# RobinVogel/Trade-offs-in-Distributed-Tuplewise-Estimation-and-Learning

Hardware: AMD Instinct MI355X
Metric: pair comparisons/sec (node) for sharded AUC U-stat at n=1e6/class (UnN, N=64 prop-SWOR shards, device repartition each step) (higher is better)
Workload: dtype f64

## Files before the change

include/tuplewise.h:

```cpp
#ifndef TUPLEWISE_H
#define TUPLEWISE_H

#include <stdint.h>

#ifdef __cplusplus
extern "C" {
#endif

#define TW_OK 0
#define TW_ERR_ARG 1
#define TW_ERR_HIP 2

#define TW_F64 0
#define TW_I64 1

#define TW_PRED_GT 0
#define TW_PRED_HALF 1
#define TW_PRED_SUBGT 2

#define TW_KERN_PROD 0
#define TW_KERN_GINI 1
#define TW_KERN_HINGE 2
#define TW_KERN_LOGISTIC 3

// ... 47 lines not shown
                  int32_t steps, int64_t x_shard, int64_t z_shard, int32_t n_shards,
                  void* d_x_bag, void* d_z_bag, uint32_t* d_cursors, uint64_t* d_send,
                  int64_t cap, int32_t* d_flag, void* stream);
int tw_chain_emit_ws(const uint64_t* d_x_rec, int64_t n_x, const uint64_t* d_z_rec, int64_t n_z,
                     int32_t half, uint32_t* d_x_pos, uint32_t* d_z_pos, int32_t first,
                     int32_t rank, int32_t world, const uint64_t* keys_x, const uint64_t* keys_z,
                     int32_t steps, int64_t x_shard, int64_t z_shard, int32_t n_shards,
                     void* d_x_bag, void* d_z_bag, uint32_t* d_cursors, uint64_t* d_send,
                     int64_t cap, int32_t* d_flag, void* d_work, int64_t work_bytes,
                     void* stream);
int64_t tw_chain_emit_work_bytes(int32_t steps, int64_t NX, int64_t NZ);
int32_t tw_chain_set_emit_tables(int32_t mode);
int32_t tw_chain_emit_tables_of(int64_t n_x, int64_t n_z, int32_t world, int32_t half,
                                int32_t exchange, int32_t n_shards);
int tw_chain_unpack(const uint64_t* d_recv, int32_t world, int32_t steps, int64_t cap,
                    int32_t half, int64_t n_x, int64_t n_z, int64_t x_shard, int64_t z_shard,
                    int32_t n_shards, void* d_x_bag, void* d_z_bag, uint32_t* d_cursors,
                    int32_t* d_flag, void* stream);
int tw_count_pairs_chain(const void* d_x_bag, const int64_t* d_x_off, int64_t x_stride,
                         const void* d_z_bag, const int64_t* d_z_off, int64_t z_stride,
                         int32_t n_shards, int32_t steps, int64_t max_nx, int64_t max_nz,
                         int32_t half, uint64_t* d_out, void* stream);
int tw_count_pairs_chain_planes(const void* d_x_bag, const int64_t* d_x_off, int64_t x_stride,
                                const void* d_z_bag, const int64_t* d_z_off, int64_t z_stride,
                                int32_t n_shards, int32_t steps, int64_t max_nx, int64_t max_nz,
                                int32_t half, int64_t image_bound, uint64_t* d_out,
                                void* stream, void* d_work, int64_t work_bytes);
int64_t tw_chain_planes_work_bytes(int32_t n_shards, int32_t steps, int64_t max_nx,
                                   int64_t max_nz, int32_t half, int64_t image_bound);
int32_t tw_count_chain_class_form(int32_t nb, int32_t k);
int32_t tw_count_chain_class_span(int32_t runs);
int32_t tw_count_chain_class_digits(int32_t w);
int32_t tw_count_chain_class_digits_of(int32_t nb, int32_t k);
int32_t tw_count_chain_prepass(int32_t mode);
int32_t tw_count_chain_prepass_of(int32_t n_shards, int32_t steps, int64_t max_nx,
                                  int64_t max_nz, int64_t image_bound);
int tw_count_pairs_chain_bucket(const void* d_x_bag, const int64_t* d_x_off, int64_t x_stride,
                                const void* d_z_bag, const int64_t* d_z_off, int64_t z_stride,
                                int32_t n_shards, int32_t steps, int64_t max_nz,
                                int64_t z_total, int32_t half, uint64_t* d_out, void* stream);
int tw_chain_set_emit(int32_t epr, int32_t steps_per_round);
int tw_count_chain_set_plan(int32_t R, int64_t z_chunk);
int tw_count_chain_set_swap(int32_t swap);
int tw_count_chain_set_class_bits(int32_t k);
int tw_chain_scatter(const void* d_x, const uint32_t* d_x_pos, int64_t n_x, const void* d_z,
                     const uint32_t* d_z_pos, int64_t n_z, void* d_x_out, void* d_z_out,
                     void* stream);

int64_t tw_count_pairs_sorted_work_bytes(int32_t n_shards, int64_t max_nz);
int tw_count_sorted_set_chunk(int64_t cap);
int tw_count_pairs_sorted(const void* d_x, const int64_t* d_x_off, const void* d_z,
                          const int64_t* d_z_off, int32_t n_shards, int64_t max_nx,
                          int64_t max_nz, int32_t dtype, int32_t pred, void* d_work,
                          uint64_t* d_out, void* stream);
int64_t tw_pair_moments_work_bytes(int32_t n_shards, int64_t total_nx, int64_t total_nz);
int tw_pair_moments(const void* d_x, const int64_t* d_x_off, const void* d_z,
                    const int64_t* d_z_off, int32_t n_shards, int64_t max_nx, int64_t max_nz,
                    int32_t dtype, int32_t pred, void* d_work, uint64_t* d_out, void* stream);
#define TW_MOMENTS_SORTED_MIN_PAIRS (1 << 17)
int tw_pair_moments_set_algo(int32_t algo);

int tw_count_pairs_sorted_step(const void* d_x, const int64_t* d_x_off, const void* d_z,
                               const int64_t* d_z_off, int32_t n_shards, int64_t max_nx,
                               int64_t max_nz, int32_t dtype, int32_t pred, void* d_work,
                               uint64_t* d_out, int64_t n_x, void* d_x_next, uint64_t key_x,
                               int64_t n_z, void* d_z_next, uint64_t key_z,
// ... 469 lines not shown
```

trade-offs-in-distributed-tuplewise-estimation-and-learning_amd/_lib.py:

```python
from __future__ import annotations

import ctypes
import os
import pathlib
import sys

import numpy as np

_HERE = pathlib.Path(__file__).resolve().parent
LIB_PATH = pathlib.Path(os.environ["TW_LIB_PATH"]) if os.environ.get("TW_LIB_PATH") else (
    _HERE / "libtuplewise.so")

TW_OK, TW_ERR_ARG, TW_ERR_HIP = 0, 1, 2
TW_F64, TW_I64 = 0, 1
TW_PRED_GT, TW_PRED_HALF, TW_PRED_SUBGT = 0, 1, 2
TW_KERN_PROD, TW_KERN_GINI, TW_KERN_HINGE, TW_KERN_LOGISTIC = 0, 1, 2, 3
TW_LOSS_HINGE, TW_LOSS_LOGISTIC = 0, 1
TW_SELF_GINI, TW_SELF_VAR, TW_SELF_KENDALL = 0, 1, 2
TW_MMD_GAUSSIAN, TW_MMD_ENERGY = 0, 1
TW_HSIC_GAUSSIAN, TW_HSIC_DISTANCE = 0, 1
TW_DIST_WITHIN, TW_DIST_CROSS = 0, 1

_vp, _i64, _i32, _u64, _f64 = (ctypes.c_void_p, ctypes.c_int64, ctypes.c_int32,
                               ctypes.c_uint64, ctypes.c_double)
# ... 194 lines not shown
    "tw_words_checksum": [_vp, _i64, _vp, _i64, _vp, _vp, _vp, _i64, _i64, _vp],
    "tw_words_checksum_acc_words": [],
    "tw_np_shuffle_pair": [_vp, _vp, _vp, _i64, _i64, _vp, _i64, _i64, _vp],
    "tw_np_shuffle_draws32": [_vp, _vp, _i64, _vp],
    "tw_np_shuffle_draws32_range": [_vp, _vp, _i64, _i64, _i64, _vp],
    "tw_shuffle_swaps_work_bytes": [_i64, _i64],
    "tw_shuffle_swaps_rounds": [_i64, _i64],
    "tw_shuffle_swaps_set_rounds": [_i32],
    "tw_shuffle_swaps_set_tail": [_i32],
    "tw_shuffle_swaps": [_vp, _i64, _vp, _i64, _vp, _vp, _i32, _i32, _vp, _vp, _vp],
    "tw_shuffle_swaps_windows": [],
    "tw_shuffle_swaps_part": [_vp, _i64, _vp, _i64, _vp, _vp, _i32, _i32, _i32, _vp, _vp, _vp],
    "tw_mt_minpoly": [_vp],
    "tw_mt_jump_poly": [_i64, _vp],
    "tw_mt_poly_mulmod": [_vp, _vp, _vp],
    "tw_mt_jump_host": [_vp, _vp, _i64],
    "tw_mt_states": [_vp, _i32, _vp, _i32, _vp, _vp],
    "tw_mt_generate": [_vp, _i32, _i32, _i32, _vp, _vp, _vp, _vp, _vp],
    "tw_np_randint_dev_work_bytes": [_i32, _i32, _i32, _i32],
    "tw_np_randint_dev": [_vp, _vp, _vp, _i32, _i32, _i32, _vp, _vp, _vp, _vp, _i32, _vp, _vp,
                          _vp, _i64, _vp, _vp, _vp],
    "tw_self_pairs_work_bytes": [_i32, _i64],
    "tw_self_pairs_idx_work_bytes": [_i32, _i64],
    "tw_self_pairs_tile": [],
    "tw_self_pairs": [_vp, _vp, _i32, _i64, _i32, _i32, _vp, _vp, _vp],
    "tw_self_pairs_idx32": [_vp, _vp, _vp, _vp, _i32, _i64, _i32, _i32, _vp, _vp, _vp],
    "tw_self_sorted_work_bytes": [_i32, _i64, _i64, _i32, _i32],
    "tw_self_sorted_chunk": [],
    "tw_self_sorted": [_vp, _vp, _i32, _i64, _i64, _i32, _i32, _i32, _vp, _vp, _vp],
    "tw_count_chain_class_form": [_i32, _i32],
    "tw_count_chain_class_span": [_i32],
    "tw_count_chain_class_digits": [_i32],
    "tw_count_chain_class_digits_of": [_i32, _i32],
    "tw_count_chain_prepass": [_i32],
    "tw_count_chain_prepass_of": [_i32, _i32, _i64, _i64, _i64],
    "tw_triplet_rows_tile": [],
    "tw_triplet_rows": [_vp, _vp, _i32, _vp, _vp, _i32, _i32, _i64, _i64, _i64, _i64, _vp, _vp,
                        _vp, _vp, _vp],
    "tw_triplet_idx_work_bytes": [_i32, _i64],
    "tw_triplet_idx32": [_vp, _vp, _i32, _vp, _vp, _vp, _vp, _i32, _i64, _i32, _vp, _vp, _vp],
    "tw_triplet_grad_tile": [],
    "tw_triplet_grad_work_bytes": [_i32, _i64, _i32, _i32],
    "tw_triplet_grad": [_vp, _vp, _i32, _vp, _i32, _vp, _vp, _vp, _vp, _i32, _i64, _f64, _i32, _vp,
                        _vp, _vp, _vp, _vp],
    "tw_triplet_project": [_vp, _i64, _i32, _vp, _i32, _vp, _vp],
    "tw_triplet_sgd_update": [_vp, _vp, _vp, _i32, _f64, _f64, _i32, _vp],
    "tw_mmd_tile": [],
    "tw_mmd_work_bytes": [_i32, _i64, _i64],
    "tw_mmd_idx_work_bytes": [_i32, _i64],
    "tw_mmd_sums": [_vp, _vp, _i32, _vp, _vp, _i32, _i64, _i64, _i32, _f64, _vp, _vp, _vp],
    "tw_mmd_idx32": [_vp, _vp, _i32, _vp, _vp, _vp, _vp, _vp, _i32, _i64, _i32, _f64, _vp, _vp,
                     _vp],
    "tw_mmd_perm_cols": [],
    "tw_mmd_perm_work_bytes": [_i64, _i32],
    "tw_mmd_perm_sums": [_vp, _i64, _i32, _vp, _i32, _i32, _f64, _vp, _vp, _vp],
    "tw_mmd_rows_max_sigma": [],
    "tw_mmd_rows_work_bytes": [_i32, _i64, _i64, _i32],
    "tw_mmd_rows": [_vp, _vp, _i32, _vp, _vp, _i32, _i64, _i64, _i32, _vp, _i32, _vp, _vp, _vp,
                    _vp],
    "tw_hsic_tile": [],
    "tw_hsic_work_bytes": [_i32, _i64, _i32],
    "tw_hsic_idx_work_bytes": [_i32, _i64],
    "tw_hsic_sums": [_vp, _i32, _vp, _i32, _vp, _i32, _i64, _i32, _f64, _f64, _i32, _vp, _vp, _vp,
                     _vp],
    "tw_hsic_idx32": [_vp, _i32, _vp, _i32, _vp, _vp, _vp, _vp, _vp, _i32, _i64, _i32, _f64, _f64,
                      _vp, _vp, _vp],
# ... 177 lines not shown
```

trade-offs-in-distributed-tuplewise-estimation-and-learning_amd/csrc/chain.hip:

```cpp
#include "bitcount.h"
#include "chainclass.h"
#include "chainplan.h"
#include "feistel.h"
#include "pkcount.h"
#include "records.h"

namespace tw {

constexpr int kChainMax = 32;
constexpr int kEmThreads = 256;
static int g_emit_epr = 0, g_emit_s = 0;
constexpr int kEmMaxB = 2 * kEmThreads;
constexpr int kEmMaxBig = 8192;

struct ChainKeys {
  uint64_t kx[kChainMax], kz[kChainMax];
};

struct ChainEmit {
  const uint64_t* xr;
  const uint64_t* zr;
  int64_t nx, nz;
  uint32_t* xpos;
  uint32_t* zpos;
// ... 571 lines not shown
      const int ng = __builtin_amdgcn_readfirstlane(it.ng);
      unsigned long long t;
      if (ng == 4)
        t = bits_count_planes<NB, 4>(pw, sf, ns, it.swapped, lane);
      else if (ng == 3)
        t = bits_count_planes<NB, 3>(pw, sf, ns, it.swapped, lane);
      else if (ng == 2)
        t = bits_count_planes<NB, 2>(pw, sf, ns, it.swapped, lane);
      else
        t = bits_count_planes<NB, 1>(pw, sf, ns, it.swapped, lane);
      tot = wave_sum_u64(t);
    }
  }
  count_chain_epilogue(tot, active, v, wid, lane, out);
}

__device__ __forceinline__ uint32_t class_block_scan(uint32_t v, uint32_t* wsum, int lane,
                                                     int wid) {
#pragma unroll
  for (int o = 1; o < kWave; o <<= 1) {
    const uint32_t t = __shfl_up(v, o, kWave);
    if (lane >= o) v += t;
  }
  if (lane == kWave - 1) wsum[wid] = v;
  __syncthreads();
  uint32_t add = 0;
  for (int w = 0; w < wid; ++w) add += wsum[w];
  __syncthreads();
  return v + add;
}

__device__ __forceinline__ uint32_t class_store_word(uint32_t zc, const ClassPlan& cp) {
  return cp.digits <= 0                 ? zc
         : cp.dbits == kClassWideBits ? class_wide_encode(zc)
                                      : class_digit_encode(zc, cp.digits);
}

struct ClassStoreForm {
  bool plain;
  int sh[kClassDigits];
  uint32_t mk[kClassDigits];
};
__device__ __forceinline__ ClassStoreForm class_store_form(const ClassPlan& cp) {
  ClassStoreForm e{};
  e.plain = cp.digits <= 0;
  const bool wide = cp.dbits == kClassWideBits;
  const int nl = e.plain ? kClassDigitMaxNL : cp.digits;
#pragma unroll
  for (int j = 0; j < kClassDigits; ++j) {
    e.sh[j] = wide ? kClassWideBits * j : class_digit_shift(nl, j);
    e.mk[j] = wide ? (j < kClassWideDigits ? (1u << kClassWideBits) - 1u : 0u)
                   : (1u << class_digit_width(nl, j)) - 1u;
  }
  return e;
}
__device__ __forceinline__ uint32_t class_store_word(uint32_t zc, const ClassStoreForm& e) {
  uint32_t w = 0;
#pragma unroll
  for (int j = 0; j < kClassDigits; ++j) w |= ((zc >> e.sh[j]) & e.mk[j]) << (8 * j);
  return e.plain ? zc : w;
}

template <bool SMALL = false>
__device__ __forceinline__ void class_block_tables(uint32_t* hist, uint32_t* wsum, int v,
                                                   const ClassPlan& cp,
                                                   uint32_t* __restrict__ work) {
  const int t = threadIdx.x, lane = t & (kWave - 1), wid = t / kWave;
  const uint32_t n = hist[t];
  const uint32_t nr = (uint32_t)class_runs(n, cp.chunk);
  const uint32_t c0 = class_block_scan(n, wsum, lane, wid) - n;
  const uint32_t e1 = class_block_scan(nr, wsum, lane, wid), e0 = e1 - nr;
  hist[t] = c0;
  if (t == kBlock - 1) work[cp.off_cnt + v] = e1;
  uint32_t* __restrict__ tab = work + (cp.off_tab + (int64_t)v * 2 * cp.cap);
  for (uint32_t j = 0; j < nr; ++j) {
    const ClassRun r =
        SMALL ? class_run32(c0, n, nr, j, (uint32_t)t) : class_run(c0, n, nr, j, (uint32_t)t);
    tab[2 * (e0 + j)] = class_entry_lo(r);
    tab[2 * (e0 + j) + 1] = class_entry_hi(r);
  }
  __syncthreads();
}

__device__ __forceinline__ void chain_zclasses_stream(const float* __restrict__ src, int64_t nz,
                                                      int v, int nb, const ClassPlan& cp,
                                                      uint32_t* hist, uint32_t* wsum,
                                                      uint32_t* __restrict__ work) {
  const int t = threadIdx.x;
  hist[t] = 0;
  __syncthreads();
  constexpr int U = 8;
  for (int64_t i0 = t; i0 < nz; i0 += kBlock * U) {
// ... 140 lines not shown
          work + bits_uniform(cp.off_tab + ((int64_t)v * cp.cap + sp.e0) * 2);
      const uint32_t* __restrict__ pw =
          work + bits_uniform(planes_word(NB, (int64_t)v * p.gx + g0, 0, 0));
      const uint32_t* __restrict__ zbag =
          work + bits_uniform(cp.off_zs + (int64_t)v * cp.zs_stride);
      unsigned long long t;
      if constexpr (DW == kClassWideBits) {
        static_assert(class_wide_fit(NB - K), "the wide digits take the 12-plane low field");
        t = bits_count_span_wide_of<NB, K, kClassDigitsMaxR>(pw, zbag, tab, sp.e1 - sp.e0, lane,
                                                             ng);
      } else if constexpr (class_loop_form(NB, K) == 3) {
        t = bits_count_span_digits_of<NB, K, kClassDigitsMaxR>(
            pw, zbag, tab, sp.e1 - sp.e0, lane, ng);
      } else {
        const ClassRun r = class_entry((uint32_t)__builtin_amdgcn_readfirstlane((int)tab[0]),
                                       (uint32_t)__builtin_amdgcn_readfirstlane((int)tab[1]));
        const uint32_t* __restrict__ zs = zbag + r.z0;
        const int len = (int)r.len;
        if (ng == 4)
          t = bits_count_class<NB, K, 4>(pw, zs, len, r.cls, lane);
        else if (ng == 3)
          t = bits_count_class<NB, K, 3>(pw, zs, len, r.cls, lane);
        else if (ng == 2)
          t = bits_count_class<NB, K, 2>(pw, zs, len, r.cls, lane);
        else
          t = bits_count_class<NB, K, 1>(pw, zs, len, r.cls, lane);
      }
      tot = wave_sum_u64(t);
    }
  }
  count_chain_epilogue(tot, active, v, wid, lane, out);
}

template <int NB>
__global__ __launch_bounds__(kBlock) void k_count_chain_swapped(
    const float* __restrict__ xb, const int64_t* __restrict__ x_off, int64_t x_stride,
    const int64_t* __restrict__ z_off, int n_shards, int n_bags, PlanesPlan p,
    const uint32_t* __restrict__ work, unsigned long long* __restrict__ out) {
  const int lb = xcd_block(blockIdx.x, gridDim.x);
  const int wid = __builtin_amdgcn_readfirstlane(threadIdx.x / kWave);
  const int lane = threadIdx.x & (kWave - 1);
  const int item = lb * (kBlock / kWave) + wid;
  const int n_swapped = p.tiles_s * p.schunks;
  const int v = item / n_swapped;
  bool active = v < n_bags;
  unsigned long long tot = 0;
  if (active) {
    const int c = v / n_shards, s = v - c * n_shards;
    const int64_t nx = x_off[s + 1] - x_off[s], nz = z_off[s + 1] - z_off[s];
    const PlanesItem it =
        planes_item(p, nx, nz, p.tiles_x * p.zchunks + (item - v * n_swapped));
    active = it.active;
    if (active) {
      const int64_t group = (int64_t)n_bags * p.gx + (int64_t)v * p.gz + it.g0;
      const uint32_t* __restrict__ pw = work + bits_uniform(planes_word(NB, group, 0, 0));
      const float* __restrict__ sf = xb + bits_uniform((int64_t)c * x_stride + x_off[s] + it.s0);
      const int ns = __builtin_amdgcn_readfirstlane((int)(it.s1 - it.s0));
      const int ng = __builtin_amdgcn_readfirstlane(it.ng);
      unsigned long long t;
      if (ng == 4)
        t = bits_count_planes<NB, 4>(pw, sf, ns, true, lane);
      else if (ng == 3)
        t = bits_count_planes<NB, 3>(pw, sf, ns, true, lane);
      else if (ng == 2)
        t = bits_count_planes<NB, 2>(pw, sf, ns, true, lane);
      else
// ... 103 lines not shown
      } else {
        *flag = 1;
      }
    }
  }
}

__global__ __launch_bounds__(kBlock) void k_chain_scatter(const uint64_t* __restrict__ xin,
                                                          const uint32_t* __restrict__ xpos,
                                                          int64_t nx,
                                                          const uint64_t* __restrict__ zin,
                                                          const uint32_t* __restrict__ zpos,
                                                          int64_t nz, uint64_t* __restrict__ xout,
                                                          uint64_t* __restrict__ zout) {
  for (int64_t e = (int64_t)blockIdx.x * kBlock + threadIdx.x; e < nx + nz;
       e += (int64_t)gridDim.x * kBlock) {
    if (e < nx)
      xout[xpos[e]] = xin[e];
    else
      zout[zpos[e - nx]] = zin[e - nx];
  }
}

struct ChainPlan {
  int R, tiles_x, zchunks;
  int64_t z_chunk, blocks;
};
static int g_chain_R = 0;
static int64_t g_chain_zchunk = 0;
static int g_planes_swap = 1;
static int g_class_bits = -1;
static int g_class_span = 0;
static int g_class_digits = 0;
static int g_prepass = 0;
static int chain_class_bits(int64_t max_nz, int64_t bags, int nb) {
  return g_class_bits < 0 ? class_bits_auto(max_nz, bags, nb)
                          : std::min(g_class_bits, std::min(kClassMaxBits, nb - 8));
}

constexpr int64_t kChainItems = 256 * 4 * 150;
constexpr int64_t kChainMinZ = 600;
static ChainPlan plan_chain(int64_t max_nx, int64_t max_nz, int64_t n_bags, bool half) {
  ChainPlan p{half ? 8 : 16, 1, 1, max_nz, 0};
  int64_t best = -1;
  if (!half) {
    for (int R : {16, 8}) {
      if (g_chain_R && R != g_chain_R) continue;
      const int64_t slots = ceil_div(max_nx, (int64_t)kWave * R) * kWave * R;
      if (best < 0 || slots < best) {
        best = slots;
        p.R = R;
      }
    }
  }
  p.tiles_x = (int)ceil_div(max_nx, (int64_t)kWave * p.R);
  const int64_t base = (int64_t)p.tiles_x * n_bags;
  int64_t zc = g_chain_zchunk;
  if (zc <= 0)
    zc = std::max<int64_t>(
        kChainMinZ, ceil_div(max_nz, std::max<int64_t>(1, ceil_div(kChainItems,
                                                                   std::max<int64_t>(1, base)))));
  zc = std::min<int64_t>(zc, (int64_t)1 << 24);
  p.z_chunk = ceil_div(std::min<int64_t>(zc, max_nz), 8) * 8;
  p.zchunks = (int)ceil_div(max_nz, p.z_chunk);
  p.blocks = ceil_div((int64_t)p.tiles_x * p.zchunks * n_bags, kBlock / kWave);
  return p;
// ... 459 lines not shown
static void count_chain_launch_planes(const PlanesPlan& p, const ClassPlan& cp, bool fused,
                                      const float* xb,
                                      const int64_t* d_x_off, int64_t x_stride, const float* zb,
                                      const int64_t* d_z_off, int64_t z_stride, int n_shards,
                                      int bags, uint32_t* work, unsigned long long* o,
                                      hipStream_t st) {
  if (fused) {
    hipLaunchKernelGGL((k_chain_prepass<NB>),
                       dim3((unsigned)prepass_grid(bags, p.gx, p.gz).blocks), dim3(kBlock), 0, st,
                       xb, d_x_off, x_stride, zb, d_z_off, z_stride, n_shards, bags, p.gx, p.gz,
                       p.swap, cp, work, o);
  } else {
    const int64_t pre = ceil_div((int64_t)bags * (p.gx + p.gz), kBlock / kWave);
    hipLaunchKernelGGL((k_chain_planes<NB>), dim3((unsigned)pre), dim3(kBlock), 0, st, xb,
                       d_x_off, x_stride, zb, d_z_off, z_stride, n_shards, bags, p.gx, p.gz,
                       p.swap, work);
  }
  if (cp.k > 0) {
    if (!fused)
      hipLaunchKernelGGL(k_chain_zclasses, dim3((unsigned)bags), dim3(kBlock), 0, st, zb, d_z_off,
                         z_stride, n_shards, bags, NB, cp, work);
    const int n_swapped = p.tiles_s * p.schunks;
    if (n_swapped > 0)
      hipLaunchKernelGGL((k_count_chain_swapped<NB>),
                         dim3((unsigned)ceil_div((int64_t)bags * n_swapped, kBlock / kWave)),
                         dim3(kBlock), 0, st, xb, d_x_off, x_stride, d_z_off, n_shards, bags, p,
                         (const uint32_t*)work, o);
    const dim3 g((unsigned)ceil_div(
                     (int64_t)bags * p.tiles_x * class_spans(cp.cap, cp.span), kBlock / kWave)),
        b(kBlock);
#define TW_CLASS_CASE(K)                                                                       \
  case K:                                                                                      \
    if constexpr (class_wide_fit(NB - K)) {                                                    \
      if (cp.dbits == kClassWideBits) {                                                        \
        hipLaunchKernelGGL((k_count_chain_classes<NB, K, kClassWideBits>), g, b, 0, st,        \
                           d_x_off, d_z_off, n_shards, bags, p, cp, (const uint32_t*)work, o); \
        break;                                                                                 \
      }                                                                                        \
    }                                                                                          \
    hipLaunchKernelGGL((k_count_chain_classes<NB, K>), g, b, 0, st, d_x_off, d_z_off,          \
                       n_shards, bags, p, cp, (const uint32_t*)work, o);                       \
    break;
    switch (cp.k) {
      TW_CLASS_CASE(1) TW_CLASS_CASE(2) TW_CLASS_CASE(3) TW_CLASS_CASE(4)
      TW_CLASS_CASE(5) TW_CLASS_CASE(6) TW_CLASS_CASE(7) TW_CLASS_CASE(8)
    }
#undef TW_CLASS_CASE
    return;
  }
  const int64_t blocks = ceil_div((int64_t)bags * p.per_bag, kBlock / kWave);
  hipLaunchKernelGGL((k_count_chain_planes<NB>), dim3((unsigned)blocks), dim3(kBlock), 0, st, xb,
                     d_x_off, x_stride, zb, d_z_off, z_stride, n_shards, bags, p,
                     (const uint32_t*)work, o);
}

static int64_t chain_planes_work_bytes(int64_t bags, int64_t max_nx, int64_t max_nz,
                                       int32_t half, int64_t image_bound) {
  const int nb = half ? 0 : bits_pick_nb(image_bound);
  if (nb == 0 || bags == 0 || max_nx == 0 || max_nz == 0) return 0;
  return (planes_work_words(max_nx, max_nz, bags, nb) + class_work_words(max_nz, bags)) *
         (int64_t)sizeof(uint32_t);
}

static int count_chain_launch_work(const void* d_x_bag, const int64_t* d_x_off, int64_t x_stride,
                                   const void* d_z_bag, const int64_t* d_z_off, int64_t z_stride,
                                   int32_t n_shards, int32_t steps, int64_t max_nx,
                                   int64_t max_nz, int32_t half, int64_t image_bound,
                                   uint64_t* d_out, void* d_work, hipStream_t st,
                                   bool zero_out) {
  const int64_t bags = (int64_t)n_shards * steps;
  const int nb = bits_pick_nb(image_bound);
  const bool sliced =
      max_nx != 0 && max_nz != 0 && chain_count_sliced(max_nx, g_chain_R, half != 0, nb);
  const int k = sliced ? chain_class_bits(max_nz, bags, nb) : 0;
  const bool fused = prepass_form(g_prepass, k, max_nz) != 1;
  if (zero_out && !fused)
    TW_HIP_CHECK(tw_zero_async(d_out, 0, sizeof(uint64_t) * (size_t)bags, st));
  if (max_nx == 0 || max_nz == 0) return TW_OK;
  if (!sliced)
    return count_chain_launch(d_x_bag, d_x_off, x_stride, d_z_bag, d_z_off, z_stride, n_shards,
                              steps, max_nx, max_nz, half, d_out, st);
  const bool digits = k > 0 && class_loop_form(nb, k) == 3;
  int R = g_chain_R >= 1 && g_chain_R <= 4 ? g_chain_R : 0;
  if (digits) R = R == 0 || R > kClassDigitsMaxR ? kClassDigitsMaxR : R;
  const int dbits = digits ? class_digit_bits(nb, k, g_class_digits) : kClassDigitBits;
  const int ndigits = dbits == kClassWideBits ? kClassWideDigits : kClassDigits;
  const PlanesPlan p =
      planes_plan(max_nx, max_nz, bags, R, g_chain_zchunk,
                  class_swap_mode(g_planes_swap, max_nx, max_nz, nb, k,
                                  digits ? ndigits + 1 : 0));
  int64_t runs = 1;
  if (digits)
    runs = g_class_span > 0
               ? g_class_span
               : class_span_auto(bags, p.tiles_x, (int)class_capacity(max_nz, k, p.z_chunk));
  ClassPlan cp = class_plan(p, max_nx, max_nz, bags, nb, k, runs);
  cp.digits = digits ? nb - k : 0;
  cp.dbits = digits ? dbits : 0;
  TW_ARG_CHECK(bags * (int64_t)p.per_bag < (1ll << 31) &&
                   bags * (int64_t)(p.gx + p.gz) < (1ll << 31) &&
                   (!fused || prepass_grid_fits(bags, p.gx, p.gz)) &&
                   bags * (int64_t)cp.per_bag < (1ll << 31),
               "tw_count_pairs_chain_planes: grid too large");
  auto* o = (unsigned long long*)d_out;
  const float* xf = (const float*)d_x_bag;
  const float* zf = (const float*)d_z_bag;
  uint32_t* w = (uint32_t*)d_work;
  if (nb == 16)
    count_chain_launch_planes<16>(p, cp, fused, xf, d_x_off, x_stride, zf, d_z_off, z_stride, n_shards,
                                  (int)bags, w, o, st);
  else if (nb == 18)
    count_chain_launch_planes<18>(p, cp, fused, xf, d_x_off, x_stride, zf, d_z_off, z_stride, n_shards,
                                  (int)bags, w, o, st);
  else if (nb == 20)
    count_chain_launch_planes<20>(p, cp, fused, xf, d_x_off, x_stride, zf, d_z_off, z_stride, n_shards,
                                  (int)bags, w, o, st);
  else if (nb == 22)
    count_chain_launch_planes<22>(p, cp, fused, xf, d_x_off, x_stride, zf, d_z_off, z_stride, n_shards,
                                  (int)bags, w, o, st);
  else
    count_chain_launch_planes<24>(p, cp, fused, xf, d_x_off, x_stride, zf, d_z_off, z_stride, n_shards,
                                  (int)bags, w, o, st);
  TW_LAUNCH_CHECK();
  return TW_OK;
}
}

extern "C" int32_t tw_count_chain_class_form(int32_t nb, int32_t k) {
  return class_loop_form(nb, k);
}

extern "C" int32_t tw_count_chain_class_span(int32_t runs) {
  const int32_t before = g_class_span;
  if (runs >= 0) g_class_span = runs;
  return before;
}

extern "C" int32_t tw_count_chain_class_digits(int32_t w) {
  const int32_t before = g_class_digits;
  if (w == -1) return before;
  TW_ARG_CHECK(w == 0 || w == kClassDigitBits || w == kClassWideBits,
               "tw_count_chain_class_digits: 0 (automatic), 3, 4 or -1 (report)");
  g_class_digits = w;
  return before;
}

extern "C" int32_t tw_count_chain_class_digits_of(int32_t nb, int32_t k) {
  return k > 0 && class_loop_form(nb, k) == 3 ? class_digit_bits(nb, k, g_class_digits)
                                              : kClassDigitBits;
}

extern "C" int32_t tw_count_chain_prepass(int32_t mode) {
  const int32_t before = g_prepass;
  if (mode == -1) return before;
  TW_ARG_CHECK(mode >= 0 && mode <= 2,
               "tw_count_chain_prepass: 0 (automatic), 1 (separate), 2 (fused) or -1 (report)");
  g_prepass = mode;
  return before;
}

extern "C" int32_t tw_count_chain_prepass_of(int32_t n_shards, int32_t steps, int64_t max_nx,
                                             int64_t max_nz, int64_t image_bound) {
  if (n_shards <= 0 || steps <= 0 || max_nx <= 0 || max_nz <= 0) return 0;
  const int nb = bits_pick_nb(image_bound);
  if (!chain_count_sliced(max_nx, g_chain_R, false, nb)) return 0;
  return prepass_form(g_prepass, chain_class_bits(max_nz, (int64_t)n_shards * steps, nb),
                      max_nz);
}

extern "C" int64_t tw_chain_planes_work_bytes(int32_t n_shards, int32_t steps, int64_t max_nx,
                                              int64_t max_nz, int32_t half,
                                              int64_t image_bound) {
  if (n_shards < 0 || steps < 0 || max_nx < 0 || max_nz < 0) return 0;
  return chain_planes_work_bytes((int64_t)n_shards * steps, max_nx, max_nz, half, image_bound);
}

extern "C" int tw_count_pairs_chain_planes(const void* d_x_bag, const int64_t* d_x_off,
// ... 212 lines not shown
```

trade-offs-in-distributed-tuplewise-estimation-and-learning_amd/csrc/chainclass.h:

```cpp
#pragma once
#include <stdint.h>

#include "bitcount.h"
#include "chainplan.h"

namespace tw {

constexpr int kClassMaxBits = 8;
constexpr int64_t kClassMinChunk = 8;

TW_BITS_HD uint32_t class_of(uint32_t zc, int nb, int k) {
  return (zc >> (nb - k)) & ((1u << k) - 1u);
}

template <int K>
TW_BITS_HD void class_gp(const uint32_t (&top)[K], uint32_t D, uint32_t& G, uint32_t& P) {
  const uint32_t m0 = bits_mask(D, 0);
  G = top[0] & m0;
  P = top[0] | m0;
#pragma unroll
  for (int b = 1; b < K; ++b) {
    const uint32_t m = bits_mask(D, b);
    G = bits_carry(top[b], m, G);
    P = bits_carry(top[b], m, P);
// ... 126 lines not shown
TW_BITS_HD uint32_t class_wide_of(uint32_t word, int j) {
  return (word >> (8 * j)) & ((1u << kClassWideBits) - 1u);
}

struct ClassWideTables {
  uint32_t g[kClassWideDigits][kClassWideEntries];
};
template <int J>
TW_BITS_HD void class_wide_tables_one(const uint32_t (&low)[kClassWideNL], uint32_t E,
                                      ClassWideTables& t) {
  uint32_t pl[kClassWideBits];
#pragma unroll
  for (int b = 0; b < kClassWideBits; ++b) pl[b] = low[kClassWideBits * J + b];
  class_digit_table<kClassWideBits>(pl, J == kClassWideDigits - 1 ? E : ~0u, t.g[J]);
}
TW_BITS_HD void class_wide_tables(const uint32_t (&low)[kClassWideNL], uint32_t E,
                                  ClassWideTables& t) {
  class_wide_tables_one<0>(low, E, t);
  class_wide_tables_one<1>(low, E, t);
  class_wide_tables_one<2>(low, E, t);
}
TW_BITS_HD ClassMasked class_gt32_wide(const ClassWideTables& t, uint32_t G, uint32_t word) {
  uint32_t c = t.g[0][class_wide_of(word, 0)];
  for (int j = 1; j < kClassWideDigits; ++j) {
    const uint32_t d = class_wide_of(word, j);
    c = bits_carry(t.g[j][d], t.g[j][d + 1], c);
  }
  return ClassMasked{G, c};
}
constexpr int kClassDigitsAuto = kClassWideBits;
TW_BITS_HD int class_digit_bits(int nb, int k, int setting) {
  const int want = setting == 0 ? kClassDigitsAuto : setting;
  return want == kClassWideBits && class_wide_fit(nb - k) ? kClassWideBits : kClassDigitBits;
}

struct ClassRun {
  int64_t z0, len;
  uint32_t cls;
};

TW_BITS_HD int64_t class_chunk(int64_t z_chunk) {
  return z_chunk < kClassMinChunk ? kClassMinChunk : z_chunk;
}
TW_BITS_HD int64_t class_runs(int64_t n, int64_t chunk) { return planes_ceil_div(n, chunk); }
TW_BITS_HD ClassRun class_run(int64_t c0, int64_t n, int64_t nr, int64_t j, uint32_t cls) {
  const int64_t a = j * n / nr, b = (j + 1) * n / nr;
  return ClassRun{c0 + a, b - a, cls};
}
TW_BITS_HD ClassRun class_run32(uint32_t c0, uint32_t n, uint32_t nr, uint32_t j, uint32_t cls) {
  const uint32_t a = j * n / nr, b = (j + 1) * n / nr;
  return ClassRun{(int64_t)(c0 + a), (int64_t)(b - a), cls};
}
TW_BITS_HD uint32_t class_entry_lo(const ClassRun& r) { return (uint32_t)r.z0 | (r.cls << 24); }
TW_BITS_HD uint32_t class_entry_hi(const ClassRun& r) { return (uint32_t)r.len; }
TW_BITS_HD ClassRun class_entry(uint32_t lo, uint32_t hi) {
  return ClassRun{(int64_t)(lo & 0xFFFFFFu), (int64_t)hi, lo >> 24};
}

TW_BITS_HD int64_t class_capacity(int64_t max_nz, int k, int64_t z_chunk) {
  return ((int64_t)1 << k) + planes_ceil_div(max_nz, class_chunk(z_chunk));
}

TW_BITS_HD int64_t class_table(const uint32_t* hist, int k, int64_t z_chunk, uint32_t* tab) {
  const int64_t chunk = class_chunk(z_chunk);
  int64_t c0 = 0, e = 0;
  for (uint32_t c = 0; c < (1u << k); ++c) {
// ... 549 lines not shown
    const int len = (int)run.len;
    cg += (uint32_t)len * ng;
    ConstWords p = zc + run.z0;
    ClassVec4 a, b;
#pragma unroll
    for (int u = 0; u < 4; ++u) a[u] = p[u];
    int j = 0;
    for (; j + 8 <= len; j += 8, p += 8) {
      batch(a, p + 4, b);
      batch(b, p + 8, a);
    }
    if (j + 4 <= len) {
      batch(a, p + 4, b);
      a = b, j += 4;
    }
    for (; j < len; ++j) {
      one(a[0]);
      a = a.yzww;
    }
  }
  unsigned long long tot = cg;
#pragma unroll
  for (int r = 0; r < R; ++r) tot += acc[r];
  return tot;
}
template <int NB, int K, int R>
__device__ __forceinline__ unsigned long long bits_count_span_wide_of(
    const uint32_t* __restrict__ pw, const uint32_t* __restrict__ zbag,
    const uint32_t* __restrict__ tab, int n, int lane, int ng) {
  if constexpr (R > 1)
    if (ng < R) return bits_count_span_wide_of<NB, K, R - 1>(pw, zbag, tab, n, lane, ng);
  return bits_count_span_wide<NB, K, R>(pw, zbag, tab, n, lane);
}
#endif

}
```

Before: 173800 billion.

## Add LDS-table class-count kernel with 8-bit low-digit lookup

Adds a 1024-thread kernel that precomputes the carry results for the low 8 bit-planes into a 128 KiB LDS table per block, then resolves each z value's comparison with a single LDS read plus one register-indexed 4-bit top-digit step, written in inline assembly. z words are re-encoded to carry the LDS byte offset directly. Blocks pull runs dynamically through an LDS atomic counter. An automatic heuristic turns the kernel on when the wide-digit form with R=2 applies and the grid fills the CUs well enough. The cost is occupancy (one block per CU because of the LDS use), a table build per block, and hand-pinned registers that are fragile.

```diff
diff --git a/include/tuplewise.h b/include/tuplewise.h
--- a/include/tuplewise.h
+++ b/include/tuplewise.h
@@ -103,6 +103,9 @@
 int32_t tw_count_chain_class_span(int32_t runs);
 int32_t tw_count_chain_class_digits(int32_t w);
 int32_t tw_count_chain_class_digits_of(int32_t nb, int32_t k);
+int32_t tw_count_chain_class_lds(int32_t mode);
+int32_t tw_count_chain_class_lds_of(int32_t n_shards, int32_t steps, int64_t max_nx,
+                                    int64_t max_nz, int64_t image_bound);
 int32_t tw_count_chain_prepass(int32_t mode);
 int32_t tw_count_chain_prepass_of(int32_t n_shards, int32_t steps, int64_t max_nx,
                                   int64_t max_nz, int64_t image_bound);
diff --git a/trade-offs-in-distributed-tuplewise-estimation-and-learning_amd/_lib.py b/trade-offs-in-distributed-tuplewise-estimation-and-learning_amd/_lib.py
--- a/trade-offs-in-distributed-tuplewise-estimation-and-learning_amd/_lib.py
+++ b/trade-offs-in-distributed-tuplewise-estimation-and-learning_amd/_lib.py
@@ -250,6 +250,8 @@
     "tw_count_chain_class_span": [_i32],
     "tw_count_chain_class_digits": [_i32],
     "tw_count_chain_class_digits_of": [_i32, _i32],
+    "tw_count_chain_class_lds": [_i32],
+    "tw_count_chain_class_lds_of": [_i32, _i32, _i64, _i64, _i64],
     "tw_count_chain_prepass": [_i32],
     "tw_count_chain_prepass_of": [_i32, _i32, _i64, _i64, _i64],
     "tw_triplet_rows_tile": [],
diff --git a/trade-offs-in-distributed-tuplewise-estimation-and-learning_amd/csrc/chain.hip b/trade-offs-in-distributed-tuplewise-estimation-and-learning_amd/csrc/chain.hip
--- a/trade-offs-in-distributed-tuplewise-estimation-and-learning_amd/csrc/chain.hip
+++ b/trade-offs-in-distributed-tuplewise-estimation-and-learning_amd/csrc/chain.hip
@@ -627,32 +627,40 @@
 
 __device__ __forceinline__ uint32_t class_store_word(uint32_t zc, const ClassPlan& cp) {
   return cp.digits <= 0                 ? zc
+         : cp.dbits == kClassLdsBits  ? class_lds_encode(zc)
          : cp.dbits == kClassWideBits ? class_wide_encode(zc)
                                       : class_digit_encode(zc, cp.digits);
 }
 
 struct ClassStoreForm {
   bool plain;
-  int sh[kClassDigits];
+  int sh[kClassDigits], at[kClassDigits];
   uint32_t mk[kClassDigits];
 };
 __device__ __forceinline__ ClassStoreForm class_store_form(const ClassPlan& cp) {
   ClassStoreForm e{};
   e.plain = cp.digits <= 0;
-  const bool wide = cp.dbits == kClassWideBits;
+  const bool wide = cp.dbits == kClassWideBits, lds = cp.dbits == kClassLdsBits;
   const int nl = e.plain ? kClassDigitMaxNL : cp.digits;
 #pragma unroll
   for (int j = 0; j < kClassDigits; ++j) {
     e.sh[j] = wide ? kClassWideBits * j : class_digit_shift(nl, j);
     e.mk[j] = wide ? (j < kClassWideDigits ? (1u << kClassWideBits) - 1u : 0u)
                    : (1u << class_digit_width(nl, j)) - 1u;
+    e.at[j] = 8 * j;
+  }
+  if (lds) {
+    e.sh[0] = kClassLdsBits, e.mk[0] = (1u << kClassWideBits) - 1u, e.at[0] = 0;
+    e.sh[1] = 0, e.mk[1] = (uint32_t)(kClassLdsEntries - 1), e.at[1] = 9;
+#pragma unroll
+    for (int j = 2; j < kClassDigits; ++j) e.sh[j] = 0, e.mk[j] = 0u, e.at[j] = 0;
   }
   return e;
 }
 __device__ __forceinline__ uint32_t class_store_word(uint32_t zc, const ClassStoreForm& e) {
   uint32_t w = 0;
 #pragma unroll
-  for (int j = 0; j < kClassDigits; ++j) w |= ((zc >> e.sh[j]) & e.mk[j]) << (8 * j);
+  for (int j = 0; j < kClassDigits; ++j) w |= ((zc >> e.sh[j]) & e.mk[j]) << e.at[j];
   return e.plain ? zc : w;
 }
 
@@ -859,6 +867,51 @@
   count_chain_epilogue(tot, active, v, wid, lane, out);
 }
 
+constexpr int kClassLdsThreads = 1024;
+constexpr int kClassLdsWaves = kClassLdsThreads / kWave;
+static_assert(kClassLdsWaves * 16 == kClassLdsEntries, "wave w writes the 16 entries d1 = w");
+static_assert(kClassLdsTableBytes + kClassLdsWaves * 8 + 8 <= 160 * 1024, "the CU's LDS");
+template <int NB, int K>
+__global__ __launch_bounds__(kClassLdsThreads) void k_count_chain_classes_lds(
+    const int64_t* __restrict__ x_off, const int64_t* __restrict__ z_off, int n_shards,
+    int n_bags, PlanesPlan p, ClassPlan cp, const uint32_t* __restrict__ work,
+    unsigned long long* __restrict__ out) {
+  __shared__ uint2 table[kClassLdsEntries * kWave];
+  __shared__ unsigned long long part[kClassLdsWaves];
+  __shared__ uint32_t next;
+  static_assert(sizeof(table) == kClassLdsTableBytes, "chainclass.h's layout");
+  const int lb = xcd_block(blockIdx.x, gridDim.x);
+  const int wid = __builtin_amdgcn_readfirstlane(threadIdx.x / kWave);
+  const int lane = threadIdx.x & (kWave - 1);
+  const int v = lb / p.tiles_x, tx = lb - v * p.tiles_x;
+  const int s = v % n_shards;
+  const int64_t nx = x_off[s + 1] - x_off[s], nz = z_off[s + 1] - z_off[s];
+  const PlanesBag bag = planes_bag(nx, nz, p.swap != 0);
+  const int lim = bag.xgroups < p.gx ? bag.xgroups : p.gx;
+  const int g0 = tx * p.R;
+  const int ng = __builtin_amdgcn_readfirstlane(lim - g0 < p.R ? lim - g0 : p.R);
+  const int cnt = __builtin_amdgcn_readfirstlane((int)work[cp.off_cnt + v]);
+  if (v >= n_bags || ng <= 0 || cnt <= 0) return;
+  const uint32_t* __restrict__ tab = work + bits_uniform(cp.off_tab + (int64_t)v * cp.cap * 2);
+  const uint32_t* __restrict__ pw =
+      work + bits_uniform(planes_word(NB, (int64_t)v * p.gx + g0, 0, 0));
+  const uint32_t* __restrict__ zbag = work + bits_uniform(cp.off_zs + (int64_t)v * cp.zs_stride);
+  if (threadIdx.x == 0) next = 0;
+  class_lds_build<NB>(table, pw, wid, lane, ng);
+  __syncthreads();
+  const uint32_t lds = (uint32_t)(uintptr_t)(__attribute__((address_space(3))) uint2*)table;
+  const unsigned long long t =
+      wave_sum_u64(bits_count_runs_lds<NB, K>(lds, pw, zbag, tab, cnt, &next, lane, ng));
+  if (lane == 0) part[wid] = t;
+  __syncthreads();
+  if (threadIdx.x == 0) {
+    unsigned long long sum = 0;
+#pragma unroll
+    for (int w = 0; w < kClassLdsWaves; ++w) sum += part[w];
+    if (sum) atomicAdd(out + v, sum);
+  }
+}
+
 template <int NB>
 __global__ __launch_bounds__(kBlock) void k_count_chain_swapped(
     const float* __restrict__ xb, const int64_t* __restrict__ x_off, int64_t x_stride,
@@ -1028,6 +1081,7 @@
 static int g_class_bits = -1;
 static int g_class_span = 0;
 static int g_class_digits = 0;
+static int g_class_lds = 0;
 static int g_prepass = 0;
 static int chain_class_bits(int64_t max_nz, int64_t bags, int nb) {
   return g_class_bits < 0 ? class_bits_auto(max_nz, bags, nb)
@@ -1553,6 +1607,13 @@
 #define TW_CLASS_CASE(K)                                                                       \
   case K:                                                                                      \
     if constexpr (class_wide_fit(NB - K)) {                                                    \
+      if (cp.dbits == kClassLdsBits) {          \
+        hipLaunchKernelGGL((k_count_chain_classes_lds<NB, K>),                                 \
+                           dim3((unsigned)((int64_t)bags * p.tiles_x)), dim3(kClassLdsThreads), \
+                           0, st, d_x_off, d_z_off, n_shards, bags, p, cp,                     \
+                           (const uint32_t*)work, o);                                          \
+        break;                                                                                 \
+      }                                                                                        \
       if (cp.dbits == kClassWideBits) {                                                        \
         hipLaunchKernelGGL((k_count_chain_classes<NB, K, kClassWideBits>), g, b, 0, st,        \
                            d_x_off, d_z_off, n_shards, bags, p, cp, (const uint32_t*)work, o); \
@@ -1581,6 +1642,15 @@
   if (nb == 0 || bags == 0 || max_nx == 0 || max_nz == 0) return 0;
   return (planes_work_words(max_nx, max_nz, bags, nb) + class_work_words(max_nz, bags)) *
          (int64_t)sizeof(uint32_t);
+}
+
+static PlanesPlan chain_digits_plan(int64_t max_nx, int64_t max_nz, int64_t bags, int nb, int k,
+                                    int dbits) {
+  int R = g_chain_R >= 1 && g_chain_R <= 4 ? g_chain_R : 0;
+  R = R == 0 || R > kClassDigitsMaxR ? kClassDigitsMaxR : R;
+  const int ndigits = dbits == kClassWideBits ? kClassWideDigits : kClassDigits;
+  return planes_plan(max_nx, max_nz, bags, R, g_chain_zchunk,
+                     class_swap_mode(g_planes_swap, max_nx, max_nz, nb, k, ndigits + 1));
 }
 
 static int count_chain_launch_work(const void* d_x_bag, const int64_t* d_x_off, int64_t x_stride,
@@ -1602,14 +1672,12 @@
     return count_chain_launch(d_x_bag, d_x_off, x_stride, d_z_bag, d_z_off, z_stride, n_shards,
                               steps, max_nx, max_nz, half, d_out, st);
   const bool digits = k > 0 && class_loop_form(nb, k) == 3;
-  int R = g_chain_R >= 1 && g_chain_R <= 4 ? g_chain_R : 0;
-  if (digits) R = R == 0 || R > kClassDigitsMaxR ? kClassDigitsMaxR : R;
   const int dbits = digits ? class_digit_bits(nb, k, g_class_digits) : kClassDigitBits;
-  const int ndigits = dbits == kClassWideBits ? kClassWideDigits : kClassDigits;
   const PlanesPlan p =
-      planes_plan(max_nx, max_nz, bags, R, g_chain_zchunk,
-                  class_swap_mode(g_planes_swap, max_nx, max_nz, nb, k,
-                                  digits ? ndigits + 1 : 0));
+      digits ? chain_digits_plan(max_nx, max_nz, bags, nb, k, dbits)
+             : planes_plan(max_nx, max_nz, bags, g_chain_R >= 1 && g_chain_R <= 4 ? g_chain_R : 0,
+                           g_chain_zchunk,
+                           class_swap_mode(g_planes_swap, max_nx, max_nz, nb, k, 0));
   int64_t runs = 1;
   if (digits)
     runs = g_class_span > 0
@@ -1617,7 +1685,7 @@
                : class_span_auto(bags, p.tiles_x, (int)class_capacity(max_nz, k, p.z_chunk));
   ClassPlan cp = class_plan(p, max_nx, max_nz, bags, nb, k, runs);
   cp.digits = digits ? nb - k : 0;
-  cp.dbits = digits ? dbits : 0;
+  cp.dbits = !digits ? 0 : class_lds_runs(g_class_lds, dbits, p, bags) ? kClassLdsBits : dbits;
   TW_ARG_CHECK(bags * (int64_t)p.per_bag < (1ll << 31) &&
                    bags * (int64_t)(p.gx + p.gz) < (1ll << 31) &&
                    (!fused || prepass_grid_fits(bags, p.gx, p.gz)) &&
@@ -1664,6 +1732,28 @@
                "tw_count_chain_class_digits: 0 (automatic), 3, 4 or -1 (report)");
   g_class_digits = w;
   return before;
+}
+
+extern "C" int32_t tw_count_chain_class_lds(int32_t mode) {
+  const int32_t before = g_class_lds;
+  if (mode == -1) return before;
+  TW_ARG_CHECK(mode >= 0 && mode <= 2,
+               "tw_count_chain_class_lds: 0 (automatic), 1 (off), 2 (on) or -1 (report)");
+  g_class_lds = mode;
+  return before;
+}
+
+extern "C" int32_t tw_count_chain_class_lds_of(int32_t n_shards, int32_t steps, int64_t max_nx,
+                                               int64_t max_nz, int64_t image_bound) {
+  if (n_shards <= 0 || steps <= 0 || max_nx <= 0 || max_nz <= 0) return 0;
+  const int64_t bags = (int64_t)n_shards * steps;
+  const int nb = bits_pick_nb(image_bound);
+  if (!chain_count_sliced(max_nx, g_chain_R, false, nb)) return 0;
+  const int k = chain_class_bits(max_nz, bags, nb);
+  if (k <= 0 || class_loop_form(nb, k) != 3) return 0;
+  const int dbits = class_digit_bits(nb, k, g_class_digits);
+  const PlanesPlan p = chain_digits_plan(max_nx, max_nz, bags, nb, k, dbits);
+  return class_lds_runs(g_class_lds, dbits, p, bags) ? 1 : 0;
 }
 
 extern "C" int32_t tw_count_chain_class_digits_of(int32_t nb, int32_t k) {
diff --git a/trade-offs-in-distributed-tuplewise-estimation-and-learning_amd/csrc/chainclass.h b/trade-offs-in-distributed-tuplewise-estimation-and-learning_amd/csrc/chainclass.h
--- a/trade-offs-in-distributed-tuplewise-estimation-and-learning_amd/csrc/chainclass.h
+++ b/trade-offs-in-distributed-tuplewise-estimation-and-learning_amd/csrc/chainclass.h
@@ -182,6 +182,52 @@
 TW_BITS_HD int class_digit_bits(int nb, int k, int setting) {
   const int want = setting == 0 ? kClassDigitsAuto : setting;
   return want == kClassWideBits && class_wide_fit(nb - k) ? kClassWideBits : kClassDigitBits;
+}
+
+constexpr int kClassLdsBits = 8;
+constexpr int kClassLdsGroups = 2;
+constexpr int kClassLdsEntries = 1 << kClassLdsBits;
+constexpr int kClassLdsEntryBytes = 64 * 4 * kClassLdsGroups;
+constexpr int kClassLdsTableBytes = kClassLdsEntries * kClassLdsEntryBytes;
+constexpr uint32_t kClassLdsOffsetMask = (uint32_t)(kClassLdsEntries - 1) * kClassLdsEntryBytes;
+static_assert(kClassLdsEntryBytes == 512 && kClassLdsTableBytes == 131072 &&
+                  kClassLdsOffsetMask == 0x1FE00u,
+              "the constants named in the loop's statements");
+TW_BITS_HD uint32_t class_lds_encode(uint32_t zc) {
+  return ((zc >> kClassLdsBits) & ((1u << kClassWideBits) - 1u)) |
+         ((zc & (uint32_t)(kClassLdsEntries - 1)) << 9);
+}
+TW_BITS_HD uint32_t class_lds_top(uint32_t word) { return word & ((1u << kClassWideBits) - 1u); }
+TW_BITS_HD uint32_t class_lds_offset(uint32_t word) { return word & kClassLdsOffsetMask; }
+TW_BITS_HD uint32_t class_lds_decode(uint32_t word) {
+  return (class_lds_top(word) << kClassLdsBits) | (class_lds_offset(word) / kClassLdsEntryBytes);
+}
+TW_BITS_HD uint32_t class_lds_entry(const ClassWideTables& t, uint32_t d8) {
+  const uint32_t d0 = d8 & 15u, d1 = (d8 >> 4) & 15u;
+  return bits_carry(t.g[1][d1], t.g[1][d1 + 1], t.g[0][d0]);
+}
+TW_BITS_HD ClassMasked class_gt32_lds(uint32_t c_low, const uint32_t (&top)[kClassWideEntries],
+                                      uint32_t G, uint32_t word) {
+  const uint32_t d = class_lds_top(word);
+  return ClassMasked{G, bits_carry(top[d], top[d + 1], c_low)};
+}
+constexpr int kClassLdsOverReadWords = 8;
+static_assert(kClassLdsOverReadWords < 64, "the over-read must stay inside the count region");
+constexpr bool class_lds_fit(int nl) { return class_wide_fit(nl); }
+constexpr int64_t kClassLdsCus = 256, kClassLdsMinBlocks = 192;
+TW_BITS_HD bool class_lds_auto(int64_t blocks) {
+  if (blocks < kClassLdsMinBlocks) return false;
+  const int64_t rounds = planes_ceil_div(blocks, kClassLdsCus);
+  const int64_t last = blocks - (rounds - 1) * kClassLdsCus;
+  if (rounds == 2) return 2 * last >= kClassLdsCus;
+  if (rounds == 3) return 4 * last >= kClassLdsCus;
+  return true;
+}
+TW_BITS_HD bool class_lds_runs(int mode, int dbits, const PlanesPlan& p, int64_t n_bags) {
+  if (mode == 1 || dbits != kClassWideBits || p.R != kClassLdsGroups ||
+      p.tiles_s * p.schunks != 0)
+    return false;
+  return mode == 2 || class_lds_auto(n_bags * p.tiles_x);
 }
 
 struct ClassRun {
@@ -797,6 +843,152 @@
     if (ng < R) return bits_count_span_wide_of<NB, K, R - 1>(pw, zbag, tab, n, lane, ng);
   return bits_count_span_wide<NB, K, R>(pw, zbag, tab, n, lane);
 }
+
+constexpr int kClassLdsTopBase0 = 24, kClassLdsTopBase1 = 42;
+static_assert(kClassLdsTopBase0 + kClassWideEntries - 1 == 40 && kClassLdsTopBase1 % 2 == 0 &&
+                  kClassLdsTopBase1 > 40 && kClassLdsTopBase1 + kClassWideEntries - 1 == 58,
+              "the registers named below");
+static_assert(kClassLdsOverReadWords == 8, "the loop's eight-word loads");
+#define TW_LD_RD(Z, A, C) \
+  "s_and_b32 s56, " Z ", 0x1fe00\n\tv_add_u32 " A ", s56, %[l8]\n\tds_read_b64 " C ", " A "\n\t"
+#define TW_LD_OPS(C0, C1) TW_DG_OP(C0, "v24", "v25") TW_DG_OP(C1, "v42", "v43")
+#define TW_LD_CNT(C0, C1) TW_DG_CNT(C0, "%[n0]") TW_DG_CNT(C1, "%[n1]")
+#define TW_LD_READS(Z0, Z1, Z2, Z3, P0, P1, P2, P3) \
+  TW_LD_RD(Z0, "v4", P0) TW_LD_RD(Z1, "v5", P1) TW_LD_RD(Z2, "v4", P2) TW_LD_RD(Z3, "v5", P3)
+#define TW_LD_CHAINS(Z0, Z1, Z2, Z3, C0, C1, C2, C3, C4, C5, C6, C7)          \
+  "s_set_gpr_idx_on " Z0 ", 0x3\n\t" TW_LD_OPS(C0, C1)                        \
+  "s_set_gpr_idx_idx " Z1 "\n\t" TW_LD_OPS(C2, C3)                            \
+  "s_set_gpr_idx_idx " Z2 "\n\t" TW_LD_OPS(C4, C5)                            \
+  "s_set_gpr_idx_idx " Z3 "\n\t" TW_LD_OPS(C6, C7) "s_set_gpr_idx_off\n\t"    \
+  TW_LD_CNT(C0, C1) TW_LD_CNT(C2, C3) TW_LD_CNT(C4, C5) TW_LD_CNT(C6, C7)
+#define TW_LD_ONE(Z)                                                          \
+  TW_LD_RD(Z, "v4", "v[8:9]") "s_waitcnt lgkmcnt(0)\n\ts_set_gpr_idx_on " Z ", 0x3\n\t" \
+  TW_LD_OPS("v8", "v9") "s_set_gpr_idx_off\n\t" TW_LD_CNT("v8", "v9")
+#define TW_LD_W0 "s40", "s41", "s42", "s43"
+#define TW_LD_W1 "s44", "s45", "s46", "s47"
+#define TW_LD_N0 "s48", "s49", "s50", "s51"
+#define TW_LD_SET_A "v8", "v9", "v10", "v11", "v12", "v13", "v14", "v15"
+#define TW_LD_SET_B "v16", "v17", "v18", "v19", "v20", "v21", "v22", "v23"
+#define TW_LD_PAIRS_A "v[8:9]", "v[10:11]", "v[12:13]", "v[14:15]"
+#define TW_LD_PAIRS_B "v[16:17]", "v[18:19]", "v[20:21]", "v[22:23]"
+#define TW_LD_X(M, ...) M(__VA_ARGS__)
+#define TW_LD_W_FROM_N                                                        \
+  "s_mov_b64 s[40:41], s[48:49]\n\ts_mov_b64 s[42:43], s[50:51]\n\t"          \
+  "s_mov_b64 s[44:45], s[52:53]\n\ts_mov_b64 s[46:47], s[54:55]\n\t"
+#define TW_LD_RUN                                                                          \
+  "s_load_dwordx8 s[40:47], %[p], 0x0\n\ts_waitcnt lgkmcnt(0)\n\t"                         \
+  "s_cmp_lt_u32 %[rem], 4\n\ts_cbranch_scc1 3f\n\t"                                        \
+  TW_LD_X(TW_LD_READS, TW_LD_W0, TW_LD_PAIRS_A) "s_waitcnt lgkmcnt(0)\n\t"                 \
+  "s_cmp_lt_u32 %[rem], 12\n\ts_cbranch_scc1 1f\n\t"                                       \
+  "0:\n\t"          \
+  "s_load_dwordx8 s[48:55], %[p], %[off] offset:0x20\n\t"                                  \
+  TW_LD_X(TW_LD_READS, TW_LD_W1, TW_LD_PAIRS_B) TW_LD_X(TW_LD_CHAINS, TW_LD_W0, TW_LD_SET_A) \
+  "s_waitcnt lgkmcnt(0)\n\t"                                                               \
+  TW_LD_X(TW_LD_READS, TW_LD_N0, TW_LD_PAIRS_A) TW_LD_X(TW_LD_CHAINS, TW_LD_W1, TW_LD_SET_B) \
+  "s_waitcnt lgkmcnt(0)\n\t" TW_LD_W_FROM_N                                                \
+  "s_add_u32 %[off], %[off], 32\n\ts_sub_u32 %[rem], %[rem], 8\n\t"                        \
+  "s_cmp_ge_u32 %[rem], 12\n\ts_cbranch_scc1 0b\n\t"                                       \
+  "1:\n\t"                         \
+  "s_cmp_lt_u32 %[rem], 8\n\ts_cbranch_scc1 2f\n\t"                                        \
+  "s_load_dwordx8 s[48:55], %[p], %[off] offset:0x20\n\t"                                  \
+  TW_LD_X(TW_LD_READS, TW_LD_W1, TW_LD_PAIRS_B) TW_LD_X(TW_LD_CHAINS, TW_LD_W0, TW_LD_SET_A) \
+  "s_waitcnt lgkmcnt(0)\n\t" TW_LD_X(TW_LD_CHAINS, TW_LD_W1, TW_LD_SET_B) TW_LD_W_FROM_N   \
+  "s_sub_u32 %[rem], %[rem], 8\n\ts_branch 3f\n\t"                                         \
+  "2:\n\t"                                                                \
+  TW_LD_X(TW_LD_CHAINS, TW_LD_W0, TW_LD_SET_A)                                             \
+  "s_mov_b64 s[40:41], s[44:45]\n\ts_mov_b64 s[42:43], s[46:47]\n\t"                       \
+  "s_sub_u32 %[rem], %[rem], 4\n\t"                                                        \
+  "3:\n\t"                                  \
+  "s_cmp_eq_u32 %[rem], 0\n\ts_cbranch_scc1 4f\n\t" TW_LD_ONE("s40")                       \
+  "s_cmp_eq_u32 %[rem], 1\n\ts_cbranch_scc1 4f\n\t" TW_LD_ONE("s41")                       \
+  "s_cmp_eq_u32 %[rem], 2\n\ts_cbranch_scc1 4f\n\t" TW_LD_ONE("s42")                       \
+  "4:\n\ts_mov_b32 %[rem], 0"
+#define TW_LD_TAB(t16, t1)                                                    \
+  "{v[24:39]}"(t16[0]), "{v40}"(t1[0]), "{v[42:57]}"(t16[1]), "{v58}"(t1[1])
+#define TW_LD_CLOBBERS                                                                         \
+  "scc", "v4", "v5", TW_LD_SET_A, TW_LD_SET_B, TW_LD_W0, TW_LD_W1, TW_LD_N0, "s52", "s53",     \
+      "s54", "s55", "s56"
+
+template <int NB, int K>
+__device__ __forceinline__ unsigned long long bits_count_runs_lds(
+    uint32_t lds, const uint32_t* __restrict__ pw, const uint32_t* __restrict__ zbag,
+    const uint32_t* __restrict__ tab, int cnt, uint32_t* next, int lane, int ng, int wid = 0,
+    int waves = 1) {
+  constexpr int NL = NB - K, W = kClassWideBits, S = W * (kClassWideDigits - 1);
+  static_assert(class_lds_fit(NL), "the table covers the low 8 planes of a 12-plane low field");
+  typedef const __attribute__((address_space(4))) uint32_t* ConstWords;
+  const ConstWords ct = (ConstWords)(uintptr_t)tab;
+  [[maybe_unused]] const ConstWords zc = (ConstWords)(uintptr_t)zbag;
+  [[maybe_unused]] const uint32_t l8 = lds + 8u * (uint32_t)lane;
+  ClassVec16 t16[kClassLdsGroups];
+  uint32_t t1[kClassLdsGroups], acc[kClassLdsGroups] = {0u, 0u};
+  uint32_t cg = 0;
+  for (int e = wid;; e += waves) {
+    if (next != nullptr) {
+      if (lane == 0) e = (int)atomicAdd(next, 1u);
+      e = __builtin_amdgcn_readfirstlane(e);
+    }
+    if (e >= cnt) break;
+    const ClassRun run = class_entry(ct[2 * e], ct[2 * e + 1]);
+    uint32_t ngp = 0;
+    int ql = lane;
+#if defined(__HIP_DEVICE_COMPILE__)
+    asm volatile("" : "+v"(ql));
 #endif
-
-}
+#pragma unroll
+    for (int r = 0; r < kClassLdsGroups; ++r) {
+      uint32_t G, P, g[kClassWideEntries], tp[K], hp[W];
+      const bool has = r < ng;
+#pragma unroll
+      for (int b = 0; b < K; ++b) tp[b] = has ? pw[(r * NB + NL + b) * 64 + ql] : 0u;
+#pragma unroll
+      for (int b = 0; b < W; ++b) hp[b] = has ? pw[(r * NB + S + b) * 64 + ql] : 0u;
+      class_gp<K>(tp, run.cls, G, P);
+      ngp = bits_popc_add(G, ngp);
+      class_digit_table<W>(hp, class_equal_mask(G, P), g);
+#pragma unroll
+      for (int d = 0; d < (1 << W); ++d) t16[r][d] = g[d];
+      t1[r] = g[1 << W];
+    }
+    cg += (uint32_t)run.len * ngp;
+#if defined(__HIP_DEVICE_COMPILE__)
+    uint32_t rem = (uint32_t)run.len, off = 0;
+    asm volatile(TW_LD_RUN
+                 : [n0] "+v"(acc[0]), [n1] "+v"(acc[1]), [rem] "+s"(rem), [off] "+s"(off)
+                 : [p] "s"(zc + run.z0), [l8] "v"(l8), TW_LD_TAB(t16, t1)
+                 : TW_LD_CLOBBERS);
+#endif
+  }
+  return (unsigned long long)cg + acc[0] + acc[1];
+}
+
+template <int NB>
+__device__ __forceinline__ void class_lds_build(uint2* tab2, const uint32_t* __restrict__ pw,
+                                                int wid, int lane, int ng) {
+  ClassWideTables t[kClassLdsGroups];
+#pragma unroll
+  for (int r = 0; r < kClassLdsGroups; ++r) {
+    uint32_t low[kClassWideNL];
+#pragma unroll
+    for (int b = 0; b < kClassLdsBits; ++b) low[b] = r < ng ? pw[(r * NB + b) * 64 + lane] : 0u;
+#pragma unroll
+    for (int b = kClassLdsBits; b < kClassWideNL; ++b) low[b] = 0u;
+    class_wide_tables_one<0>(low, ~0u, t[r]);
+    class_wide_tables_one<1>(low, ~0u, t[r]);
+  }
+  uint32_t a[kClassLdsGroups] = {0u, 0u}, b[kClassLdsGroups] = {0u, 0u};
+#pragma unroll
+  for (int d = 0; d < kClassWideEntries; ++d)
+#pragma unroll
+    for (int r = 0; r < kClassLdsGroups; ++r) {
+      a[r] = wid == d ? t[r].g[1][d] : a[r];
+      b[r] = wid + 1 == d ? t[r].g[1][d] : b[r];
+    }
+#pragma unroll
+  for (int d0 = 0; d0 < 16; ++d0)
+    tab2[(wid * 16 + d0) * 64 + lane] =
+        make_uint2(bits_carry(a[0], b[0], t[0].g[0][d0]), bits_carry(a[1], b[1], t[1].g[0][d0]));
+}
+#endif
+
+}
```

New measurement: 206900 billion, median of 6. 19.0% higher.
